# AILab-CVC/SEED-X

Measured on AMD Instinct MI355X. Metric: end-to-end generations/sec (img-in -> txt + 1024px-img-out), higher is better.
Workload: dtype fp16

## Files before the change

### seed-x_amd/csrc/gemm.hip

```cpp
#include "gemm_common.h"

namespace sxk_gemm {

template <typename TT, int BM, int BN, int WM, int WN, int NSTAGE, int AMODE>
__global__ __launch_bounds__(WM * WN * 64) void gemm_kernel(const GemmP p) {
#if defined(__HIP_DEVICE_COMPILE__)
  typedef typename TT::vec8 vec8;
  constexpr int NW = WM * WN;
  static_assert(NW == 4 || NW == 8, "4 or 8 waves per block");
  constexpr int TM = BM / WM, TN = BN / WN;
  constexpr int FM = TM / 16, FN = TN / 16;
  constexpr bool kGlu = (FN % 2 == 0);
  constexpr int BNP = (BN + 8 * NW - 1) / (8 * NW) * (8 * NW);
  constexpr int A_PER_WAVE = BM / (8 * NW);
  constexpr int B_PER_WAVE = BNP / (8 * NW);
  constexpr int LOADS = A_PER_WAVE + B_PER_WAVE;
  constexpr int A_BYTES = BM * 128, B_BYTES = BNP * 128, STAGE = A_BYTES + B_BYTES;
  static_assert(LOADS * (NSTAGE - 1) <= 63, "vmcnt range");
  extern __shared__ __attribute__((aligned(16))) unsigned char smem[];

  const int tid = threadIdx.x, lane = tid & 63;
  const int wave = __builtin_amdgcn_readfirstlane(tid >> 6);
  const int wm = wave / WN, wn = wave % WN;
  unsigned long long t_start = 0, t_first = 0, t_main = 0;
// ... 179 lines not shown
#pragma unroll
      for (int i = 0; i + 1 < FN; i += 2) {
        if (!pair_ok[i >> 1]) continue;
        u32x2_t o[2];
#pragma unroll
        for (int h = 0; h < 2; ++h) {
          f32x4_t x = v[i + h];
          if (p.act == SX_ACT_GELU) {
            const f32x2_t g0 = gelu_erf2((f32x2_t){x[0], x[1]}), g1 = gelu_erf2((f32x2_t){x[2], x[3]});
            x = (f32x4_t){g0[0], g0[1], g1[0], g1[1]};
          } else if (p.act != SX_ACT_NONE) {
#pragma unroll
            for (int r = 0; r < 4; ++r) x[r] = apply_act(x[r], p.act);
          }
          x += rv[i + h];
          if (p.out_dtype == SX_BF16) {
            o[h][0] = pack2<BF16>(x[0], x[1]);
            o[h][1] = pack2<BF16>(x[2], x[3]);
          } else {
            o[h][0] = pack2<F16>(x[0], x[1]);
            o[h][1] = pack2<F16>(x[2], x[3]);
          }
        }
        const auto s0 = __builtin_amdgcn_permlane16_swap(o[0][0], o[1][0], false, false);
        const auto s1 = __builtin_amdgcn_permlane16_swap(o[0][1], o[1][1], false, false);
        if (!mok) continue;
        const u32x4_t w4 = {s0[0], s1[0], s0[1], s1[1]};
        const int q = lane >> 4;
        const int col = n0 + wn * TN + i * 16 + (q & 1) * 16 + (q >> 1) * 8;
        *(u32x4_t*)((unsigned short*)p.C + (size_t)m * p.ldc + col) = w4;
      }
    }
#pragma unroll
    for (int i = 0; i < FN; ++i) {
      if (wide && pair_ok[i >> 1]) continue;
      if ((kGlu && p.glu)) {
        if (i & 1) continue;
        const f32x4_t g = v[(i + 1) < FN ? (i + 1) : i];
        if (p.act == SX_ACT_GELU) {
          const f32x2_t g0 = gelu_erf2((f32x2_t){g[0], g[1]}), g1 = gelu_erf2((f32x2_t){g[2], g[3]});
          v[i][0] *= g0[0]; v[i][1] *= g0[1]; v[i][2] *= g1[0]; v[i][3] *= g1[1];
        } else {
#pragma unroll
          for (int r = 0; r < 4; ++r) v[i][r] = v[i][r] * apply_act(g[r], p.act);
        }
      } else if (p.act == SX_ACT_GELU) {
        const f32x2_t g0 = gelu_erf2((f32x2_t){v[i][0], v[i][1]}), g1 = gelu_erf2((f32x2_t){v[i][2], v[i][3]});
        v[i] = (f32x4_t){g0[0], g0[1], g1[0], g1[1]};
      } else if (p.act != SX_ACT_NONE) {
#pragma unroll
        for (int r = 0; r < 4; ++r) v[i][r] = apply_act(v[i][r], p.act);
      }
      const f32x4_t o4 = v[i] + rv[i];
      if (!(mok && nok[i])) continue;
      if (p.out_dtype == SX_F32) {
        *(f32x4_t*)((float*)p.C + (size_t)m * p.ldc + nout[i]) = o4;
      } else {
        u32x2_t o;
        if (p.out_dtype == SX_BF16) {
          o[0] = pack2<BF16>(o4[0], o4[1]);
          o[1] = pack2<BF16>(o4[2], o4[3]);
        } else {
          o[0] = pack2<F16>(o4[0], o4[1]);
          o[1] = pack2<F16>(o4[2], o4[3]);
        }
        *(u32x2_t*)((unsigned short*)p.C + (size_t)m * p.ldc + nout[i]) = o;
      }
    }
  }
  if (p.dbg) {
    asm volatile("s_waitcnt vmcnt(0)" ::: "memory");
    const unsigned long long t_end = __builtin_amdgcn_s_memtime();
    if (tid == 0) {
      unsigned long long* d = p.dbg + (size_t)blockIdx.x * 4;
      d[0] = t_start; d[1] = t_first; d[2] = t_main; d[3] = t_end;
    }
  }
#endif
}

unsigned long long* g_dbg = nullptr;
int g_gm = 0;
int g_xcd_2d = 1;

template <typename TT, int BM, int BN, int WM, int WN, int NSTAGE>
int launch_cfg(const GemmP& p0, int a_mode, hipStream_t st) {
  GemmP p = p0;
  p.dbg = g_dbg;
  const int grid = plan_grid(p, BM, BN, g_xcd_2d, g_gm);
  constexpr int NW = WM * WN;
  const size_t lds = (size_t)NSTAGE * (BM + (BN + 8 * NW - 1) / (8 * NW) * (8 * NW)) * 128;
  auto reserve = [&](const void* k, hipError_t* attr, bool* done) -> hipError_t {
    int dev = 0;
    (void)hipGetDevice(&dev);
    dev &= 15;
    if (!done[dev]) {
      attr[dev] = lds > 65536 ? hipFuncSetAttribute(k, hipFuncAttributeMaxDynamicSharedMemorySize, (int)lds) : hipSuccess;
      done[dev] = true;
    }
    return attr[dev];
  };
  if (a_mode == SX_A_LINEAR) {
    auto k = gemm_kernel<TT, BM, BN, WM, WN, NSTAGE, SX_A_LINEAR>;
    static hipError_t attr[16];
    static bool done[16];
    const hipError_t e = reserve((const void*)k, attr, done);
    SX_CHECK(e == hipSuccess, "sx_gemm: cannot reserve %zu B of LDS for the %dx%d tile: %s", lds, BM, BN, hipGetErrorString(e));
    hipLaunchKernelGGL(k, dim3(grid), dim3(NW * 64), lds, st, p);
  } else {
    auto k = gemm_kernel<TT, BM, BN, WM, WN, NSTAGE, SX_A_CONV3X3>;
    static hipError_t attr[16];
    static bool done[16];
    const hipError_t e = reserve((const void*)k, attr, done);
    SX_CHECK(e == hipSuccess, "sx_gemm: cannot reserve %zu B of LDS for the %dx%d tile: %s", lds, BM, BN, hipGetErrorString(e));
    hipLaunchKernelGGL(k, dim3(grid), dim3(NW * 64), lds, st, p);
  }
  SX_HIP_LAUNCH_CHECK();
  return SX_OK;
}

struct TileCfg { int bm, bn; bool glu_ok; int slots; float a_lin, b_lin, a_conv, b_conv; };
static const int kNumTiles = 9;
static const TileCfg kTiles[kNumTiles] = {
    {128, 128, true, 512, 7.85f, 0.01202f, 15.26f, 0.01513f},  {128, 80, false, 256, 3.45f, 0.00766f, 3.59f, 0.01135f},
    {64, 128, true, 256, 1.37f, 0.00479f, 1.63f, 0.00546f},    {64, 64, true, 256, 0.33f, 0.00301f, 0.82f, 0.00313f},
    {256, 256, true, 256, 11.34f, 0.02161f, 13.19f, 0.02365f}, {256, 320, false, 256, 17.95f, 0.02566f, 18.01f, 0.02985f},
    {256, 160, false, 256, 8.13f, 0.01579f, 9.06f, 0.01897f},  {256, 256, true, 256, 10.56f, 0.01592f, 12.81f, 0.01840f},
    {256, 320, false, 256, 13.32f, 0.01928f, 15.12f, 0.02173f}};

inline int pick_tile(int M, int N, int K, bool glu, bool conv, int force, unsigned allow = 0x7f) {
  if (force >= 0 && force < kNumTiles && (!glu || kTiles[force].glu_ok)) return force;
  int best = 2;
  float best_t = 1e30f;
  for (int c = 0; c < kNumTiles; ++c) {
    const TileCfg& t = kTiles[c];
    if (!((allow >> c) & 1u)) continue;
    if (glu && !t.glu_ok) continue;
    const long tiles = (long)((M + t.bm - 1) / t.bm) * ((N + t.bn - 1) / t.bn);
    const long rounds = (tiles + t.slots - 1) / t.slots;
    const float us = (float)rounds * (conv ? t.a_conv + t.b_conv * (float)K : t.a_lin + t.b_lin * (float)K);
    if (us < best_t) { best_t = us; best = c; }
  }
  return best;
}

}
using namespace sxk_gemm;

static int g_force_tile = -1;
extern "C" int sx_gemm_pick_tile(int M, int N, int K, int glu, int conv) {
  return sxk_gemm::pick_tile(M, N, K, glu != 0, conv != 0, -1, 0x1ff);
}

extern "C" int sx_gemm_debug_stamps(void* buf) {
  sxk_gemm::g_dbg = (unsigned long long*)buf;
  return SX_OK;
}

extern "C" int sx_gemm_force_tile(int cfg) {
  if (cfg == 100 || cfg == 101) { sxk_gemm::g_xcd_2d = cfg - 100; return SX_OK; }
  if (cfg >= 300 && cfg <= 364) { sxk_gemm::g_gm = cfg - 300; return SX_OK; }
  SX_CHECK(cfg >= -1 && cfg < kNumTiles, "sx_gemm_force_tile: %d is not -1, a tile config 0..%d, 100/101 or 300..364", cfg,
           kNumTiles - 1);
  g_force_tile = cfg;
  return SX_OK;
}

static int gemm_impl(const sx_gemm_args* a, double* gn_stats, int gn_groups, int gn_rows, int* gn_fused, const sx_gemm_ln_args* ln,
                     void* stream);

extern "C" int sx_gemm(const sx_gemm_args* a, void* stream) { return gemm_impl(a, nullptr, 0, 0, nullptr, nullptr, stream); }

extern "C" int sx_gemm_ln(const sx_gemm_args* a, const sx_gemm_ln_args* ln, void* stream) {
  SX_CHECK(ln && (ln->row_stats_in || ln->row_stats_out), "sx_gemm_ln: neither a producer nor a consumer role");
  return gemm_impl(a, nullptr, 0, 0, nullptr, ln, stream);
}

extern "C" int sx_gemm_gn(const sx_gemm_args* a, double* stats, int groups, int rows_per_sample, int* fused, void* stream) {
  SX_CHECK(stats && fused && groups > 0 && rows_per_sample > 0, "sx_gemm_gn: bad statistics arguments");
  return gemm_impl(a, stats, groups, rows_per_sample, fused, nullptr, stream);
}

static int gemm_impl(const sx_gemm_args* a, double* gn_stats, int gn_groups, int gn_rows, int* gn_fused, const sx_gemm_ln_args* ln,
                     void* stream) {
  SX_CHECK(a && a->A && a->W && a->C, "sx_gemm: null pointer");
  if (gn_fused) *gn_fused = 0;
  SX_CHECK(a->dtype == SX_F16 || a->dtype == SX_BF16, "sx_gemm: dtype must be f16/bf16");
  SX_CHECK(a->out_dtype >= SX_F16 && a->out_dtype <= SX_F32, "sx_gemm: bad out_dtype");
  SX_CHECK(a->M > 0 && a->N > 0 && a->K > 0, "sx_gemm: empty problem M=%d N=%d K=%d", a->M, a->N, a->K);
  SX_CHECK(a->K % 64 == 0, "sx_gemm: K=%d must be a multiple of 64 (pad the operand)", a->K);
  SX_CHECK(a->N % 16 == 0, "sx_gemm: N=%d must be a multiple of 16 (pad the weight)", a->N);
  SX_CHECK(!a->glu || a->N % 32 == 0, "sx_gemm: glu needs N %% 32 == 0");
  const int n_out = a->glu ? a->N / 2 : a->N;
  SX_CHECK(a->n_valid >= 0 && a->n_valid % 4 == 0 && a->n_valid <= n_out, "sx_gemm: n_valid=%d", a->n_valid);
  SX_CHECK(a->ldc >= (a->n_valid > 0 ? a->n_valid : n_out) && a->ldc % 4 == 0, "sx_gemm: ldc=%d invalid for n_out=%d",
           a->ldc, n_out);
  SX_CHECK(!a->residual || (a->ldr >= (a->n_valid > 0 ? a->n_valid : n_out) && a->ldr % 4 == 0), "sx_gemm: ldr=%d invalid", a->ldr);
  SX_CHECK(!a->bias2d || a->bias2d_rows > 0, "sx_gemm: bias2d_rows must be > 0");
  GemmP p;
  memset(&p, 0, sizeof(p));
  p.A = a->A; p.W = a->W; p.C = a->C; p.bias = a->bias; p.bias2d = a->bias2d; p.residual = a->residual;
  SX_CHECK(a->a_planes >= 0 && a->a_planes <= 2, "sx_gemm: a_planes=%d", a->a_planes);
  const int planes = a->a_planes == 2 ? 2 : 1;
  SX_CHECK(planes == 1 || (a->a_mode == SX_A_LINEAR && !ln), "sx_gemm: a_planes = 2 is for plain linear GEMMs");
  const int Kk = a->K * planes;
  p.M = a->M; p.N = a->N; p.K = Kk; p.Kw = a->K; p.ldc = a->ldc; p.ldr = a->ldr; p.res_mod = a->res_mod;
  p.n_valid = a->n_valid > 0 ? a->n_valid : n_out;
  p.bias2d_rows = a->bias2d_rows; p.out_dtype = a->out_dtype; p.act = a->act; p.glu = a->glu;
  p.ldb2 = a->ld_bias2d > 0 ? a->ld_bias2d : a->N;
  p.pad = 1;
  uint64_t a_bytes;
  const bool phases = a->a_mode == SX_A_CONV3X3 && a->upsample == 2;
  if (a->a_mode == SX_A_CONV3X3) {
    SX_CHECK(a->upsample >= 0 && a->upsample <= 2, "sx_gemm conv: upsample=%d", a->upsample);
    SX_CHECK(a->Cin % 64 == 0 && a->K == (phases ? 4 : 9) * a->Cin, "sx_gemm conv: Cin=%d K=%d", a->Cin, a->K);
    SX_CHECK(a->stride == 1 || a->stride == 2, "sx_gemm conv: stride");
    if (phases) {
      SX_CHECK(a->stride == 1 && a->pad_mode == 0, "sx_gemm conv: upsample = 2 is stride 1, pad 1");
      SX_CHECK((int64_t)a->B * a->Hin * a->Win % 256 == 0,
               "sx_gemm conv: upsample = 2 needs B*Hin*Win %% 256 == 0 (B=%d Hin=%d Win=%d): a 256-row tile must not straddle a phase",
               a->B, a->Hin, a->Win);
      SX_CHECK(!a->residual && !gn_stats, "sx_gemm conv: upsample = 2 takes no residual and no GroupNorm statistics");
    }
    SX_CHECK(a->M == a->B * a->Hout * a->Wout, "sx_gemm conv: M != B*Hout*Wout");
    const int hv = a->upsample ? 2 * a->Hin : a->Hin, wv = a->upsample ? 2 * a->Win : a->Win;
    SX_CHECK(a->pad_mode == 0 || a->pad_mode == 1, "sx_gemm conv: pad_mode");
    const int padsum = a->pad_mode ? 1 : 2;
    SX_CHECK(a->Hout == (hv + padsum - 3) / a->stride + 1 && a->Wout == (wv + padsum - 3) / a->stride + 1,
             "sx_gemm conv: output geometry mismatch");
    p.pad = a->pad_mode ? 0 : 1;
    p.Hin = a->Hin; p.Win = a->Win; p.Cin = a->Cin; p.Hout = a->Hout; p.Wout = a->Wout;
    p.stride = a->stride; p.upsample = a->upsample;
    a_bytes = (uint64_t)a->B * a->Hin * a->Win * a->Cin * 2;
  } else {
    SX_CHECK(a->a_mode == SX_A_LINEAR, "sx_gemm: bad a_mode");
    a_bytes = (uint64_t)a->M * Kk * 2;
  }
  const uint64_t w_bytes = (uint64_t)a->N * a->K * 2 * (phases ? 4 : 1);
  SX_CHECK(a_bytes < 0x7fffffffull && w_bytes < 0x7fffffffull, "sx_gemm: operand exceeds 2 GiB descriptor range");
  p.a_bytes = (unsigned)a_bytes;
  p.w_bytes = (unsigned)w_bytes;
  hipStream_t st = (hipStream_t)stream;
  p.res_init = (p.residual && p.act == SX_ACT_NONE && !p.glu) ? 1 : 0;
  if (ln) {
    SX_CHECK(a->a_mode == SX_A_LINEAR && !gn_stats, "sx_gemm_ln: linear GEMMs only");
    SX_CHECK(!(ln->row_stats_in && ln->row_stats_out), "sx_gemm_ln: a launch is a producer or a consumer, not both");
// ... 49 lines not shown
```

### seed-x_amd/csrc/gemm_common.h

```cpp
#pragma once
#include "sx_common.h"

namespace sxk_gemm {

struct GemmP {
  const void* A;
  const void* W;
  void* C;
  const float* bias;
  const float* bias2d;
  const float* residual;
  int M, N, K, ldc, ldr, n_valid, res_mod, bias2d_rows, out_dtype, act, glu;
  int Kw;
  int Hin, Win, Cin, Hout, Wout, stride, upsample, ldb2, pad;
  int tiles_m, tiles_n, xm, xn;
  int gm;
  int res_init;
  unsigned a_bytes, w_bytes;
  unsigned long long* dbg;
  double* gn_stats;
  int gn_cpg, gn_groups, gn_rows;
  void* ln_x16;
  double* ln_out;
  const double* ln_in;
  const float* ln_cs;
  int ln_ldx;
  float ln_eps, ln_inv_dim;
};

template <int N>
__device__ __forceinline__ void wait_vmcnt() {
  asm volatile("s_waitcnt vmcnt(%0)" ::"n"(N) : "memory");
}

__device__ __forceinline__ bool tile_coords(const GemmP& p, int bid, int nblk, int& tile_m, int& tile_n) {
  if (p.xm == 0) {
    const int t = xcd_remap(bid, nblk);
    tile_m = t % p.tiles_m;
    tile_n = t / p.tiles_m;
    return true;
  }
  const int xcd = bid & 7, idx = bid >> 3;
  const int xr = xcd / p.xn, xc = xcd - xr * p.xn;
  const int ms = xr * p.tiles_m / p.xm, me = (xr + 1) * p.tiles_m / p.xm;
  const int ns = xc * p.tiles_n / p.xn, ne = (xc + 1) * p.tiles_n / p.xn;
  const int rm = me - ms, rn = ne - ns;
  if (idx >= rm * rn) return false;
  const int per_group = p.gm * rn;
  const int g = idx / per_group, first = g * p.gm;
  const int gsz = (rm - first) < p.gm ? (rm - first) : p.gm;
  const int r = idx - g * per_group;
  tile_m = ms + first + r % gsz;
  tile_n = ns + r / gsz;
  return true;
}

inline int plan_grid(GemmP& p, int BM, int BN, int xcd_2d, int gm_force) {
  p.tiles_m = (p.M + BM - 1) / BM;
  p.tiles_n = (p.N + BN - 1) / BN;
  int grid = p.tiles_m * p.tiles_n;
  p.xm = p.xn = 0;
  p.gm = 1;
  if (grid >= 16 && xcd_2d) {
    const double ab = (double)p.M * p.K, wb = (double)p.N * p.K;
    double best = 1e300;
    for (int xm = 1; xm <= 8; xm *= 2) {
      const int xn = 8 / xm;
      if (xm > p.tiles_m || xn > p.tiles_n) continue;
      const long padded = 8L * ((p.tiles_m + xm - 1) / xm) * ((p.tiles_n + xn - 1) / xn);
      const double cost = (ab * xn + wb * xm) * (1.0 + 4.0 * (double)(padded - grid) / grid);
      if (cost < best) { best = cost; p.xm = xm; p.xn = xn; }
    }
    if (p.xm) grid = 8 * ((p.tiles_m + p.xm - 1) / p.xm) * ((p.tiles_n + p.xn - 1) / p.xn);
    p.gm = gm_force > 0 ? gm_force : 8;
  }
  return grid;
}

int launch_pp(const GemmP& p, int dtype, int bn, int a_mode, hipStream_t st);
bool pp_supported(const GemmP& p, int dtype, int bn, int a_mode);

extern unsigned long long* g_dbg;
extern int g_gm;
extern int g_xcd_2d;

}
```

### seed-x_amd/csrc/gemm_pp.hip

```cpp
#include "gemm_common.h"
#include <type_traits>

namespace sxk_gemm {

#define SX_A_CONV3X3_UP 2
#define SX_A_CONV3X3_PH 3

#define PP_SYNC()                            \
  do {                                       \
    __builtin_amdgcn_sched_barrier(0);       \
    __builtin_amdgcn_s_barrier();            \
    __builtin_amdgcn_sched_barrier(0);       \
  } while (0)

template <typename TT, int BN, int AMODE, bool OUT32, int ACT, bool GLU, int LN = 0>
__global__ __launch_bounds__(512) void gemm_pp_kernel(const GemmP p) {
#if defined(__HIP_DEVICE_COMPILE__)
  typedef typename TT::vec8 vec8;
  static_assert(LN != 2 || (OUT32 && !GLU && ACT == SX_ACT_NONE), "the LayerNorm producer is the plain fp32-output epilogue");
  constexpr int BM = 256, TN = BN / 4, FN = TN / 16, FM = 8, FH = 4;
  constexpr int NB = BN / 64;
  constexpr int C1 = NB - 3, C2 = 3;
  constexpr int WAITN = 4 + NB;
  constexpr int A_BYTES = BM * 128, STAGE = A_BYTES + BN * 128;
  static_assert(!GLU || FN % 2 == 0, "GLU pairs n-fragments");
  static_assert(BN == 256 || BN == 320, "ping-pong tiles are 256x256 and 256x320");
  extern __shared__ __attribute__((aligned(16))) unsigned char smem[];

  const int tid = threadIdx.x, lane = tid & 63;
  const int wave = __builtin_amdgcn_readfirstlane(tid >> 6);
  const int g = wave >> 2, wc = wave & 3;
  unsigned long long t_start = 0, t_first = 0, t_main = 0;
  if (p.dbg) t_start = __builtin_amdgcn_s_memtime();

  int tile_m, tile_n;
  if (!tile_coords(p, blockIdx.x, gridDim.x, tile_m, tile_n)) return;
  const int m0 = tile_m * BM, n0 = tile_n * BN;
  const int ph = (AMODE == SX_A_CONV3X3_PH) ? m0 / (p.M >> 2) : 0;

  double ln_s1 = 0.0, ln_s2 = 0.0;
  if constexpr (LN == 1) {
    if (tid < BM) {
      const int m = m0 + tid < p.M ? m0 + tid : p.M - 1;
      ln_s1 = p.ln_in[2 * (size_t)m];
      ln_s2 = p.ln_in[2 * (size_t)m + 1];
    }
  }
  __amdgpu_buffer_rsrc_t rA = __builtin_amdgcn_make_buffer_rsrc((void*)p.A, 0, (int)p.a_bytes, 0x00020000);
  __amdgpu_buffer_rsrc_t rW = __builtin_amdgcn_make_buffer_rsrc((void*)p.W, 0, (int)p.w_bytes, 0x00020000);

  const int rl = lane >> 3;
  const unsigned gchunk = ((lane & 7) ^ rl) << 4;
  unsigned a_off[4], a_msk[4];
  int a_lrow[4];
#pragma unroll
  for (int s = 0; s < 4; ++s) {
    a_lrow[s] = g * 128 + (s >> 1) * 64 + ((2 * wave + (s & 1)) & 7) * 8;
    const int row = m0 + a_lrow[s] + rl;
    if (AMODE == SX_A_LINEAR) {
      a_off[s] = (row < p.M) ? (unsigned)row * (unsigned)p.K * 2u + gchunk : 0xC0000000u;
      a_msk[s] = 0;
    } else if (AMODE == SX_A_CONV3X3_PH) {
      const int r = row - ph * (p.M >> 2);
      const int q = r / p.Win, j = r - q * p.Win, i = q % p.Hin;
      const int sy = i + (ph >> 1) - 1, sx = j + (ph & 1) - 1;
      unsigned msk = 0;
#pragma unroll
      for (int t = 0; t < 4; ++t) {
        const int iy = sy + (t >> 1), ix = sx + (t & 1);
        if (row < p.M && iy >= 0 && iy < p.Hin && ix >= 0 && ix < p.Win) msk |= 1u << t;
      }
      a_off[s] = (unsigned)((r + ((ph >> 1) - 1) * p.Win + (ph & 1) - 1) * p.Cin) * 2u + gchunk;
      a_msk[s] = msk;
    } else {
      const int hw = p.Hout * p.Wout;
      const int b = row / hw, rem = row - b * hw;
      const int oy = rem / p.Wout, ox = rem - oy * p.Wout;
      const int Hv = p.upsample ? 2 * p.Hin : p.Hin, Wv = p.upsample ? 2 * p.Win : p.Win;
      const int vy = oy * p.stride - p.pad, vx = ox * p.stride - p.pad;
      unsigned msk = 0;
#pragma unroll
      for (int t = 0; t < 9; ++t) {
        const int iy = vy + t / 3, ix = vx + t % 3;
        if (row < p.M && iy >= 0 && iy < Hv && ix >= 0 && ix < Wv) msk |= 1u << t;
      }
      int sy = vy, sx = vx;
      if (AMODE == SX_A_CONV3X3_UP) {
        sy = oy >> 1; sx = ox >> 1;
        msk |= (unsigned)(oy & 1) << 9 | (unsigned)(ox & 1) << 10;
      }
      a_off[s] = (unsigned)(((b * p.Hin + sy) * p.Win + sx) * p.Cin) * 2u + gchunk;
      a_msk[s] = msk;
    }
  }
  unsigned w_off[NB];
  const unsigned w_ph = (unsigned)ph * (unsigned)p.N * (unsigned)p.Kw * 2u;
#pragma unroll
  for (int i = 0; i < NB; ++i) {
    const int row = n0 + (wave * NB + i) * 8 + rl;
    w_off[i] = (row < p.N) ? w_ph + (unsigned)row * (unsigned)p.Kw * 2u + gchunk : 0xC0000000u;
  }
  const int cpt = (AMODE != SX_A_LINEAR) ? p.Cin / 64 : 1;
  const int nkt = p.K / 64;
  const int nkw = p.Kw / 64;

  struct Tap { int cc, dy, dx; };
  constexpr int TW = (AMODE == SX_A_CONV3X3_PH) ? 2 : 3;
  auto tap_next = [&](Tap& t) {
    if (++t.cc == cpt) { t.cc = 0; if (++t.dx == TW) { t.dx = 0; ++t.dy; } }
  };

  auto koff_of = [&](int kt) -> unsigned { return (kt < nkt) ? (unsigned)kt * 128u : 0x80000000u; };
  auto koff_w = [&](int kt) -> unsigned { return (kt < nkt) ? (unsigned)(kt >= nkw ? kt - nkw : kt) * 128u : 0x80000000u; };
  auto dma_a = [&](int s, int buf, int kt, const Tap& t) {
    unsigned voff;
    if (AMODE == SX_A_LINEAR) {
      voff = a_off[s] + koff_of(kt);
    } else {
      const int tap = t.dy * TW + t.dx;
      const bool ok = ((a_msk[s] >> tap) & 1u) != 0 && kt < nkt;
      unsigned o;
      if (AMODE == SX_A_CONV3X3_UP) {
        const int ry = ((int)((a_msk[s] >> 9) & 1u) + t.dy - 1) >> 1, rx = ((int)((a_msk[s] >> 10) & 1u) + t.dx - 1) >> 1;
        o = a_off[s] + (unsigned)((ry * p.Win + rx) * p.Cin) * 2u + (unsigned)t.cc * 128u;
      } else {
        o = a_off[s] + (unsigned)(((t.dy * p.Win + t.dx) * p.Cin + t.cc * 64) * 2);
      }
      voff = ok ? o : 0x80000000u;
    }
    __builtin_amdgcn_raw_ptr_buffer_load_lds(rA, SX_LDS_PTR(smem + buf * STAGE + a_lrow[s] * 128), 16, voff, 0, 0, 0);
  };
  auto dma_w = [&](int i, int buf, int kt) {
    __builtin_amdgcn_raw_ptr_buffer_load_lds(rW, SX_LDS_PTR(smem + buf * STAGE + A_BYTES + (wave * NB + i) * 1024), 16,
                                             w_off[i] + koff_w(kt), 0, 0, 0);
  };
  auto issue_x = [&](int buf, int kt, const Tap& t) {
    dma_a(0, buf, kt, t);
    dma_a(1, buf, kt, t);
#pragma unroll
    for (int i = 0; i < C1; ++i) dma_w(i, buf, kt);
  };
  auto issue_y = [&](int buf, int kt) {
#pragma unroll
    for (int i = C1; i < NB; ++i) dma_w(i, buf, kt);
  };

  f32x4_t acc[FN][FM];
  const int lq = (lane >> 4) * 4;
  if (p.res_init) {
#pragma unroll
    for (int j = 0; j < FM; ++j) {
      const int m = m0 + g * 128 + j * 16 + (lane & 15);
      const int mc = m < p.M ? m : p.M - 1;
      const float* rr = p.residual + (size_t)(p.res_mod ? (mc % p.res_mod) : mc) * p.ldr;
#pragma unroll
      for (int i = 0; i < FN; ++i) {
        int c = n0 + wc * TN + i * 16 + lq;
        if (c + 4 > p.ldr) c = 0;
        acc[i][j] = *(const f32x4_t*)(rr + c);
      }
    }
  } else {
#pragma unroll
    for (int i = 0; i < FN; ++i)
#pragma unroll
      for (int j = 0; j < FM; ++j) acc[i][j] = (f32x4_t){0.f, 0.f, 0.f, 0.f};
  }

  const unsigned frag_row = (unsigned)(lane & 15) * 128u;
  unsigned frag_sw[2];
  frag_sw[0] = (unsigned)(((lane >> 4)) ^ (lane & 7)) << 4;
  frag_sw[1] = (unsigned)((4 + (lane >> 4)) ^ (lane & 7)) << 4;
  const unsigned a_frag = (unsigned)(g * 128) * 128u + frag_row;
  const unsigned w_frag = (unsigned)A_BYTES + (unsigned)(wc * TN) * 128u + frag_row;

  Tap kx = {0, 0, 0}, kz = {0, 0, 0};
  issue_x(0, 0, kx);
  issue_y(0, 0);
  dma_a(2, 0, 0, kz);
  dma_a(3, 0, 0, kz);
  tap_next(kz);
  tap_next(kx);
  issue_x(1, 1, kx);
  issue_y(1, 1);
  tap_next(kx);
  float* ln_lds = (float*)(smem + 2 * STAGE);
  if constexpr (LN == 1) {
    if (tid < BM) {
      const double mu = ln_s1 * (double)p.ln_inv_dim;
      const double var = ln_s2 * (double)p.ln_inv_dim - mu * mu;
      const float rstd = __builtin_amdgcn_rsqf((float)(var > 0.0 ? var : 0.0) + p.ln_eps);
      *(f32x2_t*)(ln_lds + 2 * tid) = (f32x2_t){rstd, -rstd * (float)mu};
    }
  }
  wait_vmcnt<WAITN>();
  PP_SYNC();
  if (p.dbg) t_first = __builtin_amdgcn_s_memtime();
  if (g == 1) PP_SYNC();

  vec8 af[FH], wf0[FN], wf1[FN];

  auto mma = [&](const vec8* wf, int h) {
    __builtin_amdgcn_s_setprio(1);
#pragma unroll
    for (int i = 0; i < FN; ++i)
#pragma unroll
      for (int j = 0; j < FH; ++j) acc[i][h * FH + j] = TT::mfma16(wf[i], af[j], acc[i][h * FH + j]);
    __builtin_amdgcn_s_setprio(0);
  };
  auto lgkm0 = [&]() { asm volatile("s_waitcnt lgkmcnt(0)" ::: "memory"); };

  auto ktile = [&](auto BUFC, int u) {
    constexpr int BUF = decltype(BUFC)::value;
    const unsigned char* sbuf = smem + BUF * STAGE;
#pragma unroll
    for (int j = 0; j < FH; ++j) af[j] = *(const vec8*)(sbuf + a_frag + j * 2048 + frag_sw[0]);
#pragma unroll
    for (int i = 0; i < FN; ++i) wf0[i] = *(const vec8*)(sbuf + w_frag + i * 2048 + frag_sw[0]);
    dma_a(2, BUF ^ 1, u + 1, kz);
    lgkm0();
    PP_SYNC();
    mma(wf0, 0);
    PP_SYNC();
#pragma unroll
    for (int j = 0; j < FH; ++j) af[j] = *(const vec8*)(sbuf + a_frag + j * 2048 + frag_sw[1]);
#pragma unroll
    for (int i = 0; i < FN; ++i) wf1[i] = *(const vec8*)(sbuf + w_frag + i * 2048 + frag_sw[1]);
    dma_a(3, BUF ^ 1, u + 1, kz);
    tap_next(kz);
    wait_vmcnt<WAITN>();
    lgkm0();
    PP_SYNC();
    mma(wf1, 0);
    PP_SYNC();
#pragma unroll
    for (int j = 0; j < FH; ++j) af[j] = *(const vec8*)(sbuf + a_frag + 8192 + j * 2048 + frag_sw[0]);
    issue_x(BUF, u + 2, kx);
    lgkm0();
    PP_SYNC();
    mma(wf0, 1);
    PP_SYNC();
#pragma unroll
    for (int j = 0; j < FH; ++j) af[j] = *(const vec8*)(sbuf + a_frag + 8192 + j * 2048 + frag_sw[1]);
    issue_y(BUF, u + 2);
    tap_next(kx);
    wait_vmcnt<WAITN>();
    lgkm0();
    PP_SYNC();
    mma(wf1, 1);
    PP_SYNC();
  };

  for (int kt = 0; kt < nkt; kt += 2) {
    ktile(std::integral_constant<int, 0>{}, kt);
    if (kt + 1 < nkt) ktile(std::integral_constant<int, 1>{}, kt + 1);
  }
  if (g == 0) PP_SYNC();
  wait_vmcnt<0>();

  if (p.dbg) t_main = __builtin_amdgcn_s_memtime();
  int ncol[FN], nout[FN];
  bool nok[FN];
  f32x4_t bv[FN];
#pragma unroll
  for (int i = 0; i < FN; ++i) {
    const int nb = n0 + wc * TN + i * 16;
    ncol[i] = nb + lq;
    nout[i] = GLU ? (nb >> 1) + lq : ncol[i];
    nok[i] = ncol[i] < p.N && nout[i] < p.n_valid && !(GLU && (i & 1));
    if (ncol[i] >= p.N) ncol[i] = p.N - 4;
    if (nout[i] + 4 > p.ldc) nout[i] = 0;
    bv[i] = (f32x4_t){0.f, 0.f, 0.f, 0.f};
  }
  if (p.bias) {
#pragma unroll
    for (int i = 0; i < FN; ++i) bv[i] = *(const f32x4_t*)(p.bias + ncol[i]);
  }
  auto out_row = [&](int m) -> int {
    if (AMODE != SX_A_CONV3X3_PH) return m;
    const int r = m - ph * (p.M >> 2);
    const int q = r / p.Win, j = r - q * p.Win;
    return (2 * q + (ph >> 1)) * p.Wout + 2 * j + (ph & 1);
  };
  const bool b2_uniform = p.bias2d && (out_row(m0) / p.bias2d_rows) == (out_row(m0 + BM - 1 < p.M ? m0 + BM - 1 : p.M - 1) / p.bias2d_rows);
  if (b2_uniform) {
    const float* b2 = p.bias2d + (size_t)(out_row(m0) / p.bias2d_rows) * p.ldb2;
#pragma unroll
    for (int i = 0; i < FN; ++i) bv[i] += *(const f32x4_t*)(b2 + ncol[i]);
  }
  const bool b2_rows = p.bias2d && !b2_uniform;
  const bool res_late = p.residual && !p.res_init;
  const bool wide = !OUT32 && !GLU && (p.ldc & 7) == 0 && (((size_t)p.C) & 15) == 0;
  bool pair_ok[(FN + 1) / 2];
#pragma unroll
  for (int i = 0; i < (FN + 1) / 2; ++i) {
    const int lim = p.n_valid < p.N ? p.n_valid : p.N;
    pair_ok[i] = (2 * i + 1 < FN) && (n0 + wc * TN + i * 32 + 32 <= lim);
  }
  const bool glu_wide = GLU && !OUT32 && (p.ldc & 7) == 0 && (((size_t)p.C) & 15) == 0 &&
                        ((n0 + wc * TN) >> 1) + 32 <= (p.n_valid < (p.N >> 1) ? p.n_valid : (p.N >> 1));
  auto act1 = [&](f32x4_t x) -> f32x4_t {
    if (ACT == SX_ACT_GELU) {
      const f32x2_t g0 = gelu_erf2((f32x2_t){x[0], x[1]}), g1 = gelu_erf2((f32x2_t){x[2], x[3]});
      return (f32x4_t){g0[0], g0[1], g1[0], g1[1]};
    } else if (ACT == SX_ACT_SILU) {
      return (f32x4_t){silu_f(x[0]), silu_f(x[1]), silu_f(x[2]), silu_f(x[3])};
    }
    return x;
  };
  auto pack4 = [&](f32x4_t x) -> u32x2_t {
    u32x2_t o;
    o[0] = pack2<TT>(x[0], x[1]);
    o[1] = pack2<TT>(x[2], x[3]);
    return o;
  };
  f32x4_t lcs[LN == 1 ? FN : 1];
  if constexpr (LN == 1) {
#pragma unroll
    for (int i = 0; i < FN; ++i) lcs[i] = *(const f32x4_t*)(p.ln_cs + ncol[i]);
  }
  float lsum[LN == 2 ? FM : 1], lsq[LN == 2 ? FM : 1];
  const bool gn = OUT32 && p.gn_stats != nullptr;
  float gsl[FN], gql[FN], gsh[FN], gqh[FN];
#pragma unroll
  for (int i = 0; i < FN; ++i) gsl[i] = gql[i] = gsh[i] = gqh[i] = 0.f;
#pragma unroll
  for (int j = 0; j < FM; ++j) {
    const int m = m0 + g * 128 + j * 16 + (lane & 15);
    const bool mok = m < p.M;
    const int mc = mok ? m : p.M - 1;
    const int mo = out_row(m);
    f32x4_t v[FN];
    if constexpr (LN == 1) {
      const f32x2_t ab = *(const f32x2_t*)(ln_lds + 2 * (g * 128 + j * 16 + (lane & 15)));
#pragma unroll
      for (int i = 0; i < FN; ++i) v[i] = acc[i][j] * ab[0] + (lcs[i] * ab[1] + bv[i]);
    } else {
#pragma unroll
      for (int i = 0; i < FN; ++i) v[i] = acc[i][j] + bv[i];
    }
    if (b2_rows) {
      const float* b2 = p.bias2d + (size_t)(out_row(mc) / p.bias2d_rows) * p.ldb2;
#pragma unroll
      for (int i = 0; i < FN; ++i) v[i] += *(const f32x4_t*)(b2 + ncol[i]);
    }
    if (GLU) {
#pragma unroll
      for (int i = 0; i + 1 < FN; i += 2) {
        const f32x4_t gt = act1(v[i + 1]);
        v[i] = v[i] * gt;
      }
    } else if (ACT != SX_ACT_NONE) {
#pragma unroll
      for (int i = 0; i < FN; ++i) v[i] = act1(v[i]);
    }
    if (res_late) {
      const float* rr = p.residual + (size_t)(p.res_mod ? (mc % p.res_mod) : mc) * p.ldr;
#pragma unroll
      for (int i = 0; i < FN; ++i) {
        if (GLU && (i & 1)) continue;
        const int c = (nout[i] + 4 <= p.ldr) ? nout[i] : 0;
        v[i] += *(const f32x4_t*)(rr + c);
      }
    }
    if (OUT32) {
#pragma unroll
      for (int i = 0; i < FN; ++i)
        if (mok && nok[i]) *(f32x4_t*)((float*)p.C + (size_t)mo * p.ldc + nout[i]) = v[i];
      if constexpr (LN == 2) {
        float s1 = 0.f, s2 = 0.f;
#pragma unroll
        for (int i = 0; i < FN; ++i) {
          if (mok && nok[i]) {
            s1 += (v[i][0] + v[i][1]) + (v[i][2] + v[i][3]);
            s2 += (v[i][0] * v[i][0] + v[i][1] * v[i][1]) + (v[i][2] * v[i][2] + v[i][3] * v[i][3]);
          }
        }
        lsum[j] = s1;
        lsq[j] = s2;
        const bool xwide = (p.ln_ldx & 7) == 0 && (((size_t)p.ln_x16) & 15) == 0;
#pragma unroll
        for (int i = 0; i < FN; ++i) {
          if ((i & 1) == 0 && i + 1 < FN && xwide && pair_ok[i >> 1]) {
            const u32x2_t o0 = pack4(v[i]), o1 = pack4(v[i + 1]);
            const auto w0 = __builtin_amdgcn_permlane16_swap(o0[0], o1[0], false, false);
            const auto w1 = __builtin_amdgcn_permlane16_swap(o0[1], o1[1], false, false);
            if (mok) {
              const u32x4_t w4 = {w0[0], w1[0], w0[1], w1[1]};
              const int q = lane >> 4;
              const int col = n0 + wc * TN + i * 16 + (q & 1) * 16 + (q >> 1) * 8;
              *(u32x4_t*)((unsigned short*)p.ln_x16 + (size_t)m * p.ln_ldx + col) = w4;
            }
            continue;
          }
          if ((i & 1) && xwide && pair_ok[i >> 1]) continue;
          if (mok && nok[i]) *(u32x2_t*)((unsigned short*)p.ln_x16 + (size_t)m * p.ln_ldx + nout[i]) = pack4(v[i]);
        }
      }
      if (gn && mok) {
#pragma unroll
        for (int i = 0; i < FN; ++i) {
          gsl[i] += v[i][0] + v[i][1];
          gql[i] += v[i][0] * v[i][0] + v[i][1] * v[i][1];
          gsh[i] += v[i][2] + v[i][3];
          gqh[i] += v[i][2] * v[i][2] + v[i][3] * v[i][3];
        }
      }
    } else {
      if constexpr (GLU && FN == 4) {
        if (glu_wide) {
          const u32x2_t o0 = pack4(v[0]), o1 = pack4(v[2]);
          const auto s0 = __builtin_amdgcn_permlane16_swap(o0[0], o1[0], false, false);
          const auto s1 = __builtin_amdgcn_permlane16_swap(o0[1], o1[1], false, false);
          if (mok) {
            const u32x4_t w4 = {s0[0], s1[0], s0[1], s1[1]};
            const int q = lane >> 4;
            const int col = ((n0 + wc * TN) >> 1) + (q & 1) * 16 + (q >> 1) * 8;
// ... 3 lines not shown
        }
      }
#pragma unroll
      for (int i = 0; i < FN; ++i) {
        if (GLU && (i & 1)) continue;
        if (!GLU && wide && (i & 1) == 0 && i + 1 < FN && pair_ok[i >> 1]) {
          const u32x2_t o0 = pack4(v[i]), o1 = pack4(v[i + 1]);
          const auto s0 = __builtin_amdgcn_permlane16_swap(o0[0], o1[0], false, false);
          const auto s1 = __builtin_amdgcn_permlane16_swap(o0[1], o1[1], false, false);
          if (mok) {
            const u32x4_t w4 = {s0[0], s1[0], s0[1], s1[1]};
            const int q = lane >> 4;
            const int col = n0 + wc * TN + i * 16 + (q & 1) * 16 + (q >> 1) * 8;
            *(u32x4_t*)((unsigned short*)p.C + (size_t)mo * p.ldc + col) = w4;
          }
          continue;
        }
        if (!GLU && wide && (i & 1) && pair_ok[i >> 1]) continue;
        if (mok && nok[i]) *(u32x2_t*)((unsigned short*)p.C + (size_t)mo * p.ldc + nout[i]) = pack4(v[i]);
      }
    }
  }
  if constexpr (LN == 2) {
    float* racc = (float*)smem;
    __syncthreads();
#pragma unroll
    for (int j = 0; j < FM; ++j) {
      float s1 = lsum[j], s2 = lsq[j];
      s1 += __shfl_xor(s1, 16, 64); s2 += __shfl_xor(s2, 16, 64);
      s1 += __shfl_xor(s1, 32, 64); s2 += __shfl_xor(s2, 32, 64);
      if (lane < 16) *(f32x2_t*)(racc + ((size_t)(wc * BM + g * 128 + j * 16 + lane)) * 2) = (f32x2_t){s1, s2};
    }
    __syncthreads();
    if (tid < BM && m0 + tid < p.M) {
      float s1 = 0.f, s2 = 0.f;
#pragma unroll
      for (int w = 0; w < 4; ++w) { s1 += racc[(w * BM + tid) * 2]; s2 += racc[(w * BM + tid) * 2 + 1]; }
      atomicAdd(&p.ln_out[2 * (size_t)(m0 + tid)], (double)s1);
      atomicAdd(&p.ln_out[2 * (size_t)(m0 + tid) + 1], (double)s2);
    }
  }
  if (OUT32 && gn) {
    auto row16_sum = [](float x) -> float {
      x += __builtin_bit_cast(float, __builtin_amdgcn_update_dpp(0, __builtin_bit_cast(int, x), 0xB1, 0xF, 0xF, true));
      x += __builtin_bit_cast(float, __builtin_amdgcn_update_dpp(0, __builtin_bit_cast(int, x), 0x4E, 0xF, 0xF, true));
      x += __builtin_bit_cast(float, __builtin_amdgcn_update_dpp(0, __builtin_bit_cast(int, x), 0x141, 0xF, 0xF, true));
      x += __builtin_bit_cast(float, __builtin_amdgcn_update_dpp(0, __builtin_bit_cast(int, x), 0x140, 0xF, 0xF, true));
      return x;
    };
#pragma unroll
    for (int i = 0; i < FN; ++i) {
      gsl[i] = row16_sum(gsl[i]);
      gql[i] = row16_sum(gql[i]);
      gsh[i] = row16_sum(gsh[i]);
      gqh[i] = row16_sum(gqh[i]);
    }
    float* gslot = (float*)smem;
    const int gbase = n0 / p.gn_cpg;
    const int nlast = (n0 + BN < p.N ? n0 + BN : p.N) - 1;
    const int ngr = nlast / p.gn_cpg - gbase + 1;
    __syncthreads();
    if ((lane & 15) == 0) {
#pragma unroll
      for (int i = 0; i < FN; ++i) {
        const int cp = (wc * TN + i * 16 + lq) >> 1;
        *(f32x4_t*)(gslot + ((size_t)g * (BN / 2) + cp) * 2) = (f32x4_t){gsl[i], gql[i], gsh[i], gqh[i]};
      }
    }
    __syncthreads();
    const int smp = m0 / p.gn_rows;
    for (int t = tid; t < 2 * ngr; t += 512) {
      const int G = gbase + (t >> 1), which = t & 1;
      int c_lo = G * p.gn_cpg - n0, c_hi = (G + 1) * p.gn_cpg - n0;
      c_lo = c_lo < 0 ? 0 : c_lo;
      const int c_end = (p.N - n0 < BN ? p.N - n0 : BN);
      c_hi = c_hi > c_end ? c_end : c_hi;
      float acc = 0.f;
      for (int cp = c_lo >> 1; cp < (c_hi >> 1); ++cp) acc += gslot[(size_t)cp * 2 + which];
      for (int cp = c_lo >> 1; cp < (c_hi >> 1); ++cp) acc += gslot[((size_t)(BN / 2) + cp) * 2 + which];
      atomicAdd(&p.gn_stats[((size_t)smp * p.gn_groups + G) * 2 + which], (double)acc);
    }
  }
  if (p.dbg) {
    asm volatile("s_waitcnt vmcnt(0)" ::: "memory");
    const unsigned long long t_end = __builtin_amdgcn_s_memtime();
    if (tid == 0) {
      unsigned long long* d = p.dbg + (size_t)blockIdx.x * 4;
      d[0] = t_start; d[1] = t_first; d[2] = t_main; d[3] = t_end;
    }
  }
#endif
}

template <typename TT, int BN, int AMODE, bool OUT32, int ACT, bool GLU, int LN = 0>
static int launch_one(const GemmP& p0, hipStream_t st) {
  GemmP p = p0;
  p.dbg = g_dbg;
  const int grid = plan_grid(p, 256, BN, g_xcd_2d, g_gm);
  constexpr size_t lds = 2 * (size_t)(256 + BN) * 128 + (LN == 1 ? 2048 : 0);
  auto k = gemm_pp_kernel<TT, BN, AMODE, OUT32, ACT, GLU, LN>;
  static hipError_t attr[16];
  static bool done[16];
  int dev = 0;
  (void)hipGetDevice(&dev);
  dev &= 15;
  if (!done[dev]) {
    attr[dev] = hipFuncSetAttribute((const void*)k, hipFuncAttributeMaxDynamicSharedMemorySize, (int)lds);
    done[dev] = true;
  }
  SX_CHECK(attr[dev] == hipSuccess, "sx_gemm: cannot reserve %zu B of LDS for the 256x%d ping-pong tile: %s", lds, BN,
           hipGetErrorString(attr[dev]));
  hipLaunchKernelGGL(k, dim3(grid), dim3(512), lds, st, p);
  SX_HIP_LAUNCH_CHECK();
  return SX_OK;
}

static int epi_code(const GemmP& p, int dtype) {
  const bool out32 = p.out_dtype == SX_F32;
  if (!out32 && p.out_dtype != dtype) return -1;
  if (p.glu) {
    if (out32) return -1;
    if (p.act == SX_ACT_GELU) return 2;
    if (p.act == SX_ACT_SILU) return 3;
    return -1;
  }
  if (p.act == SX_ACT_NONE) return out32 ? 4 : 0;
  if (p.act == SX_ACT_GELU && !out32) return 1;
  return -1;
}

bool pp_supported(const GemmP& p, int dtype, int bn, int a_mode) {
  const int e = epi_code(p, dtype);
  if (e < 0) return false;
  if (p.ln_in && !(a_mode == SX_A_LINEAR && (e == 0 || e == 2) && !p.ln_out)) return false;
  if (p.ln_out && !(a_mode == SX_A_LINEAR && e == 4 && !p.gn_stats)) return false;
  if (bn == 320 && (e == 2 || e == 3)) return false;
  if (a_mode == SX_A_CONV3X3 && !(e == 0 || e == 4)) return false;
  if (a_mode == SX_A_CONV3X3 && p.upsample && !(p.stride == 1 && p.pad == 1)) return false;
  return bn == 256 || bn == 320;
}

template <typename TT>
static int launch_phases(const GemmP& p, int e, int bn, hipStream_t st) {
#define PH_CASE(BNV, O32) return launch_one<TT, BNV, SX_A_CONV3X3_PH, O32, SX_ACT_NONE, false>(p, st)
  if (bn == 256) {
    if (e == 0) PH_CASE(256, false);
    if (e == 4) PH_CASE(256, true);
  } else {
    if (e == 0) PH_CASE(320, false);
    if (e == 4) PH_CASE(320, true);
  }
#undef PH_CASE
  return -1;
}

template <typename TT>
static int launch_t(const GemmP& p, int dtype, int bn, int a_mode, hipStream_t st) {
  const int e = epi_code(p, dtype);
  if (a_mode == SX_A_CONV3X3 && p.upsample == 2) return launch_phases<TT>(p, e, bn, st);
#define PP_CASE(BNV, AM, O32, ACTV, GLUV) return launch_one<TT, BNV, AM, O32, ACTV, GLUV>(p, st)
  if (p.ln_in) {
    if (e == 2) return launch_one<TT, 256, SX_A_LINEAR, false, SX_ACT_GELU, true, 1>(p, st);
    if (bn == 256) return launch_one<TT, 256, SX_A_LINEAR, false, SX_ACT_NONE, false, 1>(p, st);
    return launch_one<TT, 320, SX_A_LINEAR, false, SX_ACT_NONE, false, 1>(p, st);
  }
  if (p.ln_out) {
    if (bn == 256) return launch_one<TT, 256, SX_A_LINEAR, true, SX_ACT_NONE, false, 2>(p, st);
    return launch_one<TT, 320, SX_A_LINEAR, true, SX_ACT_NONE, false, 2>(p, st);
  }
  if (a_mode == SX_A_LINEAR) {
    if (bn == 256) {
      switch (e) {
        case 0: PP_CASE(256, SX_A_LINEAR, false, SX_ACT_NONE, false);
        case 1: PP_CASE(256, SX_A_LINEAR, false, SX_ACT_GELU, false);
        case 2: PP_CASE(256, SX_A_LINEAR, false, SX_ACT_GELU, true);
        case 3: PP_CASE(256, SX_A_LINEAR, false, SX_ACT_SILU, true);
        case 4: PP_CASE(256, SX_A_LINEAR, true, SX_ACT_NONE, false);
      }
    } else {
      switch (e) {
        case 0: PP_CASE(320, SX_A_LINEAR, false, SX_ACT_NONE, false);
        case 1: PP_CASE(320, SX_A_LINEAR, false, SX_ACT_GELU, false);
        case 4: PP_CASE(320, SX_A_LINEAR, true, SX_ACT_NONE, false);
      }
    }
  } else if (!p.upsample) {
    if (bn == 256) {
      switch (e) {
        case 0: PP_CASE(256, SX_A_CONV3X3, false, SX_ACT_NONE, false);
        case 4: PP_CASE(256, SX_A_CONV3X3, true, SX_ACT_NONE, false);
      }
// ... 30 lines not shown
```

Before: 1.301.

## Make ping-pong GEMM persistent, prefetching next tile during epilogue

```diff
diff --git a/seed-x_amd/csrc/gemm.hip b/seed-x_amd/csrc/gemm.hip
--- a/seed-x_amd/csrc/gemm.hip
+++ b/seed-x_amd/csrc/gemm.hip
@@ -285,6 +285,8 @@
 unsigned long long* g_dbg = nullptr;
 int g_gm = 0;
 int g_xcd_2d = 1;
+int g_walk = 1;
+int g_walk_cap = 0;
 
 template <typename TT, int BM, int BN, int WM, int WN, int NSTAGE>
 int launch_cfg(const GemmP& p0, int a_mode, hipStream_t st) {
@@ -363,8 +365,10 @@
 extern "C" int sx_gemm_force_tile(int cfg) {
   if (cfg == 100 || cfg == 101) { sxk_gemm::g_xcd_2d = cfg - 100; return SX_OK; }
   if (cfg >= 300 && cfg <= 364) { sxk_gemm::g_gm = cfg - 300; return SX_OK; }
-  SX_CHECK(cfg >= -1 && cfg < kNumTiles, "sx_gemm_force_tile: %d is not -1, a tile config 0..%d, 100/101 or 300..364", cfg,
-           kNumTiles - 1);
+  if (cfg == 700 || cfg == 701) { sxk_gemm::g_walk = cfg - 700; return SX_OK; }
+  if (cfg >= 800 && cfg <= 864) { sxk_gemm::g_walk_cap = cfg - 800; return SX_OK; }
+  SX_CHECK(cfg >= -1 && cfg < kNumTiles, "sx_gemm_force_tile: %d is not -1, a tile config 0..%d, 100/101, 300..364, 700/701 or 800..864",
+           cfg, kNumTiles - 1);
   g_force_tile = cfg;
   return SX_OK;
 }
diff --git a/seed-x_amd/csrc/gemm_common.h b/seed-x_amd/csrc/gemm_common.h
--- a/seed-x_amd/csrc/gemm_common.h
+++ b/seed-x_amd/csrc/gemm_common.h
@@ -15,6 +15,7 @@
   int Hin, Win, Cin, Hout, Wout, stride, upsample, ldb2, pad;
   int tiles_m, tiles_n, xm, xn;
   int gm;
+  int nblk;
   int res_init;
   unsigned a_bytes, w_bytes;
   unsigned long long* dbg;
@@ -74,6 +75,7 @@
     if (p.xm) grid = 8 * ((p.tiles_m + p.xm - 1) / p.xm) * ((p.tiles_n + p.xn - 1) / p.xn);
     p.gm = gm_force > 0 ? gm_force : 8;
   }
+  p.nblk = grid;
   return grid;
 }
 
@@ -83,5 +85,7 @@
 extern unsigned long long* g_dbg;
 extern int g_gm;
 extern int g_xcd_2d;
+extern int g_walk;
+extern int g_walk_cap;
 
 }
diff --git a/seed-x_amd/csrc/gemm_pp.hip b/seed-x_amd/csrc/gemm_pp.hip
--- a/seed-x_amd/csrc/gemm_pp.hip
+++ b/seed-x_amd/csrc/gemm_pp.hip
@@ -12,6 +12,10 @@
     __builtin_amdgcn_s_barrier();            \
     __builtin_amdgcn_sched_barrier(0);       \
   } while (0)
+
+__host__ __device__ constexpr bool pp_walks(int bn, int amode, bool out32, int ln) {
+  return amode == SX_A_LINEAR && !out32 && ln != 2 && !(bn == 320 && ln == 1);
+}
 
 template <typename TT, int BN, int AMODE, bool OUT32, int ACT, bool GLU, int LN = 0>
 __global__ __launch_bounds__(512) void gemm_pp_kernel(const GemmP p) {
@@ -33,30 +37,38 @@
   unsigned long long t_start = 0, t_first = 0, t_main = 0;
   if (p.dbg) t_start = __builtin_amdgcn_s_memtime();
 
+  constexpr bool WALK = pp_walks(BN, AMODE, OUT32, LN);
+  int vb = blockIdx.x;
   int tile_m, tile_n;
-  if (!tile_coords(p, blockIdx.x, gridDim.x, tile_m, tile_n)) return;
-  const int m0 = tile_m * BM, n0 = tile_n * BN;
+  if (!tile_coords(p, vb, p.nblk, tile_m, tile_n)) return;
+  int m0 = tile_m * BM, n0 = tile_n * BN;
   const int ph = (AMODE == SX_A_CONV3X3_PH) ? m0 / (p.M >> 2) : 0;
 
   double ln_s1 = 0.0, ln_s2 = 0.0;
-  if constexpr (LN == 1) {
-    if (tid < BM) {
-      const int m = m0 + tid < p.M ? m0 + tid : p.M - 1;
-      ln_s1 = p.ln_in[2 * (size_t)m];
-      ln_s2 = p.ln_in[2 * (size_t)m + 1];
-    }
-  }
+  auto ln_load = [&](int mt, int tid) {
+    if constexpr (LN == 1) {
+      if (tid < BM) {
+        const int m = mt + tid < p.M ? mt + tid : p.M - 1;
+        ln_s1 = p.ln_in[2 * (size_t)m];
+        ln_s2 = p.ln_in[2 * (size_t)m + 1];
+      }
+    }
+  };
+  ln_load(m0, tid);
   __amdgpu_buffer_rsrc_t rA = __builtin_amdgcn_make_buffer_rsrc((void*)p.A, 0, (int)p.a_bytes, 0x00020000);
   __amdgpu_buffer_rsrc_t rW = __builtin_amdgcn_make_buffer_rsrc((void*)p.W, 0, (int)p.w_bytes, 0x00020000);
 
+  unsigned a_off[4], a_msk[4];
+  int a_lrow[4];
+  unsigned w_off[NB];
+  const unsigned w_ph = (unsigned)ph * (unsigned)p.N * (unsigned)p.Kw * 2u;
+  auto lane_offsets = [&](int mt, int nt, int lane) {
   const int rl = lane >> 3;
   const unsigned gchunk = ((lane & 7) ^ rl) << 4;
-  unsigned a_off[4], a_msk[4];
-  int a_lrow[4];
 #pragma unroll
   for (int s = 0; s < 4; ++s) {
     a_lrow[s] = g * 128 + (s >> 1) * 64 + ((2 * wave + (s & 1)) & 7) * 8;
-    const int row = m0 + a_lrow[s] + rl;
+    const int row = mt + a_lrow[s] + rl;
     if (AMODE == SX_A_LINEAR) {
       a_off[s] = (row < p.M) ? (unsigned)row * (unsigned)p.K * 2u + gchunk : 0xC0000000u;
       a_msk[s] = 0;
@@ -93,13 +105,13 @@
       a_msk[s] = msk;
     }
   }
-  unsigned w_off[NB];
-  const unsigned w_ph = (unsigned)ph * (unsigned)p.N * (unsigned)p.Kw * 2u;
 #pragma unroll
   for (int i = 0; i < NB; ++i) {
-    const int row = n0 + (wave * NB + i) * 8 + rl;
+    const int row = nt + (wave * NB + i) * 8 + rl;
     w_off[i] = (row < p.N) ? w_ph + (unsigned)row * (unsigned)p.Kw * 2u + gchunk : 0xC0000000u;
   }
+  };
+  lane_offsets(m0, n0, lane);
   const int cpt = (AMODE != SX_A_LINEAR) ? p.Cin / 64 : 1;
   const int nkt = p.K / 64;
   const int nkw = p.Kw / 64;
@@ -167,36 +179,44 @@
       for (int j = 0; j < FM; ++j) acc[i][j] = (f32x4_t){0.f, 0.f, 0.f, 0.f};
   }
 
-  const unsigned frag_row = (unsigned)(lane & 15) * 128u;
-  unsigned frag_sw[2];
-  frag_sw[0] = (unsigned)(((lane >> 4)) ^ (lane & 7)) << 4;
-  frag_sw[1] = (unsigned)((4 + (lane >> 4)) ^ (lane & 7)) << 4;
-  const unsigned a_frag = (unsigned)(g * 128) * 128u + frag_row;
-  const unsigned w_frag = (unsigned)A_BYTES + (unsigned)(wc * TN) * 128u + frag_row;
+  unsigned frag_sw[2], a_frag, w_frag;
+  auto frag_offsets = [&](int lane) {
+    const unsigned frag_row = (unsigned)(lane & 15) * 128u;
+    frag_sw[0] = (unsigned)(((lane >> 4)) ^ (lane & 7)) << 4;
+    frag_sw[1] = (unsigned)((4 + (lane >> 4)) ^ (lane & 7)) << 4;
+    a_frag = (unsigned)(g * 128) * 128u + frag_row;
+    w_frag = (unsigned)A_BYTES + (unsigned)(wc * TN) * 128u + frag_row;
+  };
+  frag_offsets(lane);
 
   Tap kx = {0, 0, 0}, kz = {0, 0, 0};
-  issue_x(0, 0, kx);
-  issue_y(0, 0);
-  dma_a(2, 0, 0, kz);
-  dma_a(3, 0, 0, kz);
-  tap_next(kz);
-  tap_next(kx);
-  issue_x(1, 1, kx);
-  issue_y(1, 1);
-  tap_next(kx);
+  auto prologue = [&]() {
+    kx = kz = Tap{0, 0, 0};
+    issue_x(0, 0, kx);
+    issue_y(0, 0);
+    dma_a(2, 0, 0, kz);
+    dma_a(3, 0, 0, kz);
+    tap_next(kz);
+    tap_next(kx);
+    issue_x(1, 1, kx);
+    issue_y(1, 1);
+    tap_next(kx);
+  };
   float* ln_lds = (float*)(smem + 2 * STAGE);
-  if constexpr (LN == 1) {
-    if (tid < BM) {
-      const double mu = ln_s1 * (double)p.ln_inv_dim;
-      const double var = ln_s2 * (double)p.ln_inv_dim - mu * mu;
-      const float rstd = __builtin_amdgcn_rsqf((float)(var > 0.0 ? var : 0.0) + p.ln_eps);
-      *(f32x2_t*)(ln_lds + 2 * tid) = (f32x2_t){rstd, -rstd * (float)mu};
-    }
-  }
+  auto ln_table = [&](int which, int tid) {
+    if constexpr (LN == 1) {
+      if (tid < BM) {
+        const double mu = ln_s1 * (double)p.ln_inv_dim;
+        const double var = ln_s2 * (double)p.ln_inv_dim - mu * mu;
+        const float rstd = __builtin_amdgcn_rsqf((float)(var > 0.0 ? var : 0.0) + p.ln_eps);
+        *(f32x2_t*)(ln_lds + which * 2 * BM + 2 * tid) = (f32x2_t){rstd, -rstd * (float)mu};
+      }
+    }
+  };
+  prologue();
+  int lt = 0;
+  ln_table(lt, tid);
   wait_vmcnt<WAITN>();
-  PP_SYNC();
-  if (p.dbg) t_first = __builtin_amdgcn_s_memtime();
-  if (g == 1) PP_SYNC();
 
   vec8 af[FH], wf0[FN], wf1[FN];
 
@@ -251,6 +271,11 @@
     PP_SYNC();
   };
 
+  for (;;) {
+  PP_SYNC();
+  if (p.dbg) t_first = __builtin_amdgcn_s_memtime();
+  if (g == 1) PP_SYNC();
+
   for (int kt = 0; kt < nkt; kt += 2) {
     ktile(std::integral_constant<int, 0>{}, kt);
     if (kt + 1 < nkt) ktile(std::integral_constant<int, 1>{}, kt + 1);
@@ -259,6 +284,9 @@
   wait_vmcnt<0>();
 
   if (p.dbg) t_main = __builtin_amdgcn_s_memtime();
+  int lane_e = (int)(threadIdx.x & 63);
+  if constexpr (WALK) asm volatile("" : "+v"(lane_e));
+  const int lane = lane_e, tid = wave * 64 + lane_e, lq = (lane_e >> 4) * 4;
   int ncol[FN], nout[FN];
   bool nok[FN];
   f32x4_t bv[FN];
@@ -324,6 +352,37 @@
   float gsl[FN], gql[FN], gsh[FN], gqh[FN];
 #pragma unroll
   for (int i = 0; i < FN; ++i) gsl[i] = gql[i] = gsh[i] = gqh[i] = 0.f;
+
+  bool has_next = false;
+  int nm0 = m0, nn0 = n0;
+  if constexpr (WALK) {
+    const int nvb = vb + (int)gridDim.x;
+    int ntm, ntn;
+    if (nvb < p.nblk && tile_coords(p, nvb, p.nblk, ntm, ntn)) {
+      has_next = true;
+      nm0 = ntm * BM;
+      nn0 = ntn * BN;
+    }
+    ln_load(nm0, tid);
+    lane_offsets(nm0, nn0, lane);
+    if (!has_next) {
+#pragma unroll
+      for (int s = 0; s < 4; ++s) a_off[s] = 0xC0000000u;
+#pragma unroll
+      for (int i = 0; i < NB; ++i) w_off[i] = 0xC0000000u;
+    }
+    prologue();
+    ln_table(lt ^ 1, tid);
+    asm volatile("" ::: "memory");
+    __builtin_amdgcn_sched_barrier(0);
+  }
+  constexpr int NSTORE = GLU ? FM * (FN / 4) : FM * (FN / 2 + (FN & 1));
+  static_assert(!WALK || WAITN + NSTORE <= 63, "vmcnt is a 6-bit field on gfx9");
+  bool interior = false;
+  if constexpr (WALK) {
+    const int lim = p.n_valid < p.N ? p.n_valid : p.N;
+    interior = m0 + BM <= p.M && (GLU ? (FN == 4 && glu_wide) : (wide && n0 + wc * TN + TN <= lim));
+  }
 #pragma unroll
   for (int j = 0; j < FM; ++j) {
     const int m = m0 + g * 128 + j * 16 + (lane & 15);
@@ -332,7 +391,7 @@
     const int mo = out_row(m);
     f32x4_t v[FN];
     if constexpr (LN == 1) {
-      const f32x2_t ab = *(const f32x2_t*)(ln_lds + 2 * (g * 128 + j * 16 + (lane & 15)));
+      const f32x2_t ab = *(const f32x2_t*)(ln_lds + lt * 2 * BM + 2 * (g * 128 + j * 16 + (lane & 15)));
 #pragma unroll
       for (int i = 0; i < FN; ++i) v[i] = acc[i][j] * ab[0] + (lcs[i] * ab[1] + bv[i]);
     } else {
@@ -502,12 +561,36 @@
     }
   }
   if (p.dbg) {
-    asm volatile("s_waitcnt vmcnt(0)" ::: "memory");
+    if (!has_next) asm volatile("s_waitcnt vmcnt(0)" ::: "memory");
     const unsigned long long t_end = __builtin_amdgcn_s_memtime();
     if (tid == 0) {
-      unsigned long long* d = p.dbg + (size_t)blockIdx.x * 4;
+      unsigned long long* d = p.dbg + (size_t)vb * 4;
       d[0] = t_start; d[1] = t_first; d[2] = t_main; d[3] = t_end;
     }
+    t_start = t_main;
+  }
+  if constexpr (!WALK) {
+    break;
+  } else {
+    if (!has_next) {
+      wait_vmcnt<0>();
+      break;
+    }
+    vb += (int)gridDim.x;
+    m0 = nm0;
+    n0 = nn0;
+#pragma unroll
+    for (int i = 0; i < FN; ++i)
+#pragma unroll
+      for (int j = 0; j < FM; ++j) acc[i][j] = (f32x4_t){0.f, 0.f, 0.f, 0.f};
+    lt ^= 1;
+    int lane_m = (int)(threadIdx.x & 63);
+    asm volatile("" : "+v"(lane_m));
+    lane_offsets(m0, n0, lane_m);
+    frag_offsets(lane_m);
+    if (interior) wait_vmcnt<WAITN + NSTORE>();
+    else wait_vmcnt<WAITN>();
+  }
   }
 #endif
 }
@@ -516,17 +599,24 @@
 static int launch_one(const GemmP& p0, hipStream_t st) {
   GemmP p = p0;
   p.dbg = g_dbg;
-  const int grid = plan_grid(p, 256, BN, g_xcd_2d, g_gm);
-  constexpr size_t lds = 2 * (size_t)(256 + BN) * 128 + (LN == 1 ? 2048 : 0);
+  int grid = plan_grid(p, 256, BN, g_xcd_2d, g_gm);
+  constexpr size_t lds = 2 * (size_t)(256 + BN) * 128 + (LN == 1 ? (pp_walks(BN, AMODE, OUT32, LN) ? 2 : 1) * 2048 : 0);
   auto k = gemm_pp_kernel<TT, BN, AMODE, OUT32, ACT, GLU, LN>;
   static hipError_t attr[16];
   static bool done[16];
+  static int cus[16];
   int dev = 0;
   (void)hipGetDevice(&dev);
   dev &= 15;
   if (!done[dev]) {
     attr[dev] = hipFuncSetAttribute((const void*)k, hipFuncAttributeMaxDynamicSharedMemorySize, (int)lds);
+    if (hipDeviceGetAttribute(&cus[dev], hipDeviceAttributeMultiprocessorCount, dev) != hipSuccess) cus[dev] = 0;
     done[dev] = true;
+  }
+  if (pp_walks(BN, AMODE, OUT32, LN) && g_walk && !p.residual && !p.bias2d) {
+    int resident = 8 * (cus[dev] / 8);
+    if (g_walk_cap > 0 && 8 * g_walk_cap < resident) resident = 8 * g_walk_cap;
+    if (resident >= 8 && grid > resident) grid = resident;
   }
   SX_CHECK(attr[dev] == hipSuccess, "sx_gemm: cannot reserve %zu B of LDS for the 256x%d ping-pong tile: %s", lds, BN,
            hipGetErrorString(attr[dev]));
```

After: 1.312 (median of 6 runs). No clear change (+0.8%).
